# team-charls/charls

Hardware: AMD Instinct MI355X
Metric: MPixels/s encode+decode, 4096x4096 8-bit gray, bit-exact vs CharLS (higher is better)
Workload: dtype u8

## Files before the change

### charls_amd/csrc/device/tile_pipeline.hip

```cpp
#pragma once
#include <hip/hip_runtime.h>

#include <algorithm>
#include <cstdlib>

#include "pipeline_common.hip"

namespace jls {
namespace tile {

using pipe::kChains;
using pipe::kInterruptChain;
using pipe::kNoEvent;
using pipe::kStatusInvalid;
using pipe::kZeroContextChain;


constexpr uint32_t kMaxTileSamples = 8192;
constexpr uint32_t kTileLines = 16;
constexpr uint32_t kSegments = 16;
constexpr uint32_t kThreads = 512;
constexpr uint32_t kWaves = kThreads / 64;
constexpr uint32_t kPackThreads = 512;
constexpr uint16_t kNoLocalSlot = 0xFFFF;
template <typename S>
struct SlotOf
{
    typedef uint32_t type;
};
template <>
struct SlotOf<uint8_t>
{
    typedef uint16_t type;
};
template <typename S>
using Slot = typename SlotOf<S>::type;
template <typename S>
constexpr uint32_t run_slots_of()
{
    return sizeof(Slot<S>) == 2 ? 2u : 1u;
}
constexpr uint32_t kRowChainWords = 288;
constexpr uint32_t kChainPad = 32;
constexpr uint32_t kSlack = kChains * kChainPad + 128;
__host__ __device__ inline uint64_t slots_capacity(uint64_t samples, uint32_t run_slots, uint64_t lines)
{
    const uint64_t runs = samples / 2 + lines < samples ? samples / 2 + lines : samples;
    return samples + (run_slots > 1 ? runs : 0);
}
__host__ __device__ inline size_t stage_bytes(uint32_t tile_capacity, uint32_t sample_bytes)
{
    return sample_bytes == 1 ? (size_t)slots_capacity(tile_capacity, 2, kTileLines) * 2 : (size_t)tile_capacity * 4;
}
constexpr uint32_t kPlanGroups = 64;
#define JLS_HOST_DEV_EARLY __host__ __device__ inline
constexpr uint32_t kRunTag = 1u << 31;

enum Counter : uint32_t
{
    kCountJobs = 0,
    kCountJobsRewalked = 1,
    kCountRunJobs = 2,
    kCountRunJobsRewalked = 3,
    kCountRareSegments = 4,
    kCountRareSerial = 5,
// ... 175 lines not shown
        __syncthreads();
        if (lane == 63)
        {
            s_tmp[wave] = incl_a;
            s_tmp[kWaves + wave] = incl_b;
        }
        __syncthreads();
        uint32_t before_a = carry_a, before_b = carry_b, all_a = 0, all_b = 0;
        for (int w2 = 0; w2 < waves; ++w2)
        {
            const uint32_t na = s_tmp[w2], nb = s_tmp[kWaves + w2];
            before_a += w2 < wave ? na : 0;
            before_b += w2 < wave ? nb : 0;
            all_a += na;
            all_b += nb;
        }
        a[half] = before_a + incl_a - a[half];
        b[half] = before_b + incl_b - b[half];
        carry_a += all_a;
        carry_b += all_b;
    }
}

template <typename S, int ILV>
struct Samples
{
    const ScanDesc& d;
    const S* rows;
    uint32_t first_line;
    int mask;
    JLS_DEV int operator()(uint32_t line, uint32_t x) const
    {
        static_assert(ILV == 0, "planar scans only");
        return (int)rows[(size_t)(line + 1 - first_line) * d.width + x] & mask;
    }
};

template <typename S, int ILV>
JLS_DEV void stage_lines(const ScanDesc& d, const TileGeometry& g, S* rows)
{
    const uint32_t width = g.width;
    const uint32_t bytes = width * (uint32_t)sizeof(S);
    const uint32_t first = g.first_line == 0 ? 1u : 0u;
    if (first)
        for (uint32_t x = threadIdx.x; x < width; x += blockDim.x)
            rows[x] = 0;
// ... 69 lines not shown
__global__ void __launch_bounds__(kThreads) analyze_tiles(const ScanDesc* __restrict__ descs, const Work* __restrict__ works)
{
    JLS_DYNAMIC_LDS(smem);
    const ScanDesc d = descs[blockIdx.y];
    const Work w = works[blockIdx.y];
    const Traits t = make_traits(d);
    const uint32_t tile = tile_of_block(blockIdx.x, scan_tiles(d, w));
    if (tile >= scan_tiles(d, w))
        return;
    const TileGeometry g = tile_geometry(d, w, tile);
    constexpr uint32_t step = 1;
    const int lane = threadIdx.x & 63, wave = threadIdx.x >> 6;
    const uint32_t width = g.width, chunks = g.chunks;
    const TileLds lds = tile_lds<S, ILV>(width, w.lines_per_tile, true);
    S* s_rows = reinterpret_cast<S*>(smem + lds.rows);
    uint16_t* s_key = reinterpret_cast<uint16_t*>(smem + lds.keys);
    uint64_t* s_eq = reinterpret_cast<uint64_t*>(smem + lds.masks);
    uint64_t* s_q0 = s_eq + (size_t)w.lines_per_tile * chunks;
    uint32_t* s_hist = reinterpret_cast<uint32_t*>(smem + lds.table);
    unsigned char* s_grad = reinterpret_cast<unsigned char*>(s_hist + kChains + 1);
    const int mask = (1 << d.bits_per_sample) - 1;
    const Samples<S, ILV> sample{d, s_rows, g.first_line, mask};

    stage_lines<S, ILV>(d, g, s_rows);
    for (uint32_t c = threadIdx.x; c < (uint32_t)kChains; c += kThreads)
        s_hist[c] = 0;
    if (sizeof(S) == 1)
        for (uint32_t q = threadIdx.x; q < 511; q += kThreads)
            s_grad[q] = (unsigned char)(quantize(t, (int)q - 255) + 4);
    __syncthreads();

    for (uint32_t sgm = wave; sgm < g.segments; sgm += kWaves)
    {
        const uint32_t r = sgm / g.pieces, piece = sgm % g.pieces;
        const uint32_t y = g.first_line + r;
        const uint32_t k0 = piece * g.chunks_per_piece;
        const uint32_t k1 = k0 + g.chunks_per_piece < chunks ? k0 + g.chunks_per_piece : chunks;
        const int edge_a = y >= step ? sample(y - step, 0) : 0;
        const int edge_c = y >= 2 * step ? (r >= 1 ? sample(y - 2 * step, 0) : pipe::load_sample<S, 0>(d, y - 2, 0, mask)) : 0;
        for (uint32_t k = k0; k < k1; ++k)
        {
            const uint32_t x = k * 64 + lane;
            bool eq = false, q0 = false;
            if (x < width)
            {
                const int v = sample(y, x);
                const int ra = x > 0 ? sample(y, x - 1) : edge_a;
                int rb = 0, rc = 0, rd = 0;
                if (y >= step)
                {
                    rb = sample(y - step, x);
                    rc = x > 0 ? sample(y - step, x - 1) : edge_c;
                    rd = sample(y - step, x + 1 < width ? x + 1 : width - 1);
                }
                else
                    rc = x > 0 ? 0 : edge_c;
                const int qs = sizeof(S) == 1
                                   ? ((int)s_grad[rd - rb + 255] * 9 + (int)s_grad[rb - rc + 255]) * 9 + (int)s_grad[rc - ra + 255] - 364
                                   : context_id(t, ra, rb, rc, rd);
                const int sg = qs >> 31;
                const int ctx = (qs ^ sg) - sg;
                s_key[r * width + x] = (uint16_t)(ctx | ((sg & 1) << 9));
                eq = v == ra;
                q0 = qs == 0;
            }
            const unsigned long long m_eq = __ballot(eq);
            const unsigned long long m_q0 = __ballot(q0);
            if (lane == 0)
            {
                s_eq[r * chunks + k] = m_eq;
                s_q0[r * chunks + k] = m_q0;
            }
        }
    }
    __syncthreads();
    for (uint32_t sgm = wave; sgm < g.segments; sgm += kWaves)
    {
        const uint32_t r = sgm / g.pieces, piece = sgm % g.pieces;
        const uint32_t y = g.first_line + r;
        const uint32_t k0 = piece * g.chunks_per_piece;
        const uint32_t k1 = k0 + g.chunks_per_piece < chunks ? k0 + g.chunks_per_piece : chunks;
        const auto key_row = global_ptr(w.keyinv) + (size_t)y * width;
        unsigned long long carry = 0;
        for (uint32_t k = 0; k < k1; ++k)
        {
            const unsigned long long a = s_eq[r * chunks + k];
            const unsigned long long b = a & s_q0[r * chunks + k];
            const unsigned long long sum = a + b + carry;
            const unsigned long long st = sum ^ a ^ b;
            carry = (((a & b) | ((a | b) & st)) >> 63) & 1ull;
            const uint32_t x = k * 64 + lane;
            if (k >= k0 && x < width)
            {
                const bool s = (st >> lane) & 1ull;
                const bool q0 = (s_q0[r * chunks + k] >> lane) & 1ull;
                const bool eq = (a >> lane) & 1ull;
                uint16_t key = s_key[r * width + x];
                if (!(s || q0))
                    atomicAdd(&s_hist[key & 0x1FF], 1u);
                else if (s && eq)
                    key = kNoEvent;
                else if (s)
                {
                    key = (uint16_t)kInterruptChain;
                    atomicAdd(&s_hist[kInterruptChain], 1u);
                }
                else
                {
                    key = 0;
                    atomicAdd(&s_hist[0], 1u);
                }
                key_row[x] = key;
            }
        }
    }
    __syncthreads();
    for (uint32_t c = threadIdx.x; c < (uint32_t)kChains; c += kThreads)
        global_ptr(w.seg)[(size_t)tile * kChains + c] = s_hist[c];
}

constexpr uint32_t kPlanThreads = 384;
JLS_DEV void plan_group(const ScanDesc& d, const Work& w, uint32_t g, uint32_t& t0, uint32_t& t1)
{
    const uint32_t tiles = scan_tiles(d, w);
    const uint32_t per_group = (tiles + kPlanGroups - 1) / kPlanGroups;
    t0 = g * per_group < tiles ? g * per_group : tiles;
    t1 = t0 + per_group < tiles ? t0 + per_group : tiles;
}
__global__ void __launch_bounds__(kPlanThreads) sum_chains(const ScanDesc* __restrict__ descs, const Work* __restrict__ works)
{
    const ScanDesc d = descs[blockIdx.y];
    const Work w = works[blockIdx.y];
    const uint32_t g = blockIdx.x, c = threadIdx.x;
    if (c >= (uint32_t)kChains)
        return;
    uint32_t t0, t1;
    plan_group(d, w, g, t0, t1);
    uint32_t sum = 0;
    for (uint32_t t = t0; t < t1; ++t)
        sum += w.seg[(size_t)t * kChains + c];
    w.plan_part[g * kChains + c] = sum * (c == 0 ? w.run_slots : 1u);
// ... 105 lines not shown
    static JLS_DEV int err(uint32_t v) { return (int)(v << (32 - kRunBits - kErrBits)) >> (32 - kErrBits); }
    static JLS_DEV int which(uint32_t v) { return (int)((v >> (kRunBits + kErrBits)) & 1u); }
    static JLS_DEV uint32_t component(uint32_t v) { return (v >> (is_end_of_line(v) ? 15u : kRunBits + kErrBits + 1)) & 3u; }
};

template <typename S, int ILV>
__global__ void __launch_bounds__(kThreads) sort_tiles(const ScanDesc* __restrict__ descs, const Work* __restrict__ works)
{
    JLS_DYNAMIC_LDS(smem);
    const ScanDesc d = descs[blockIdx.y];
    const Work w = works[blockIdx.y];
    const Traits t = make_traits(d);
    const uint32_t tile = tile_of_block(blockIdx.x, scan_tiles(d, w));
    if (tile >= scan_tiles(d, w))
        return;
    const TileGeometry g = tile_geometry(d, w, tile);
    constexpr uint32_t step = 1;
    const int lane = threadIdx.x & 63, wave = threadIdx.x >> 6;
    const uint32_t width = g.width, chunks = g.chunks;
    const TileLds lds = tile_lds<S, ILV>(width, w.lines_per_tile, false);
    S* s_rows = reinterpret_cast<S*>(smem + lds.rows);
    uint64_t* s_noev = reinterpret_cast<uint64_t*>(smem + lds.masks);
    uint32_t* s_lead = reinterpret_cast<uint32_t*>(s_noev + (size_t)w.lines_per_tile * chunks);
    uint32_t* s_segoff = reinterpret_cast<uint32_t*>(smem + lds.table);
    uint32_t* s_tileoff = s_segoff + sort_segments(w.lines_per_tile) * kChains;
    uint32_t* s_count = s_tileoff + kChains + 1;
    uint32_t* s_global = s_count + kChains + 1;
    uint32_t* s_tmp = s_global + kChains + 1;
    uint32_t* s_same = s_tmp + 16;
    uint32_t* s_rowbase = s_same + kWaves * (kChains + 1);
    uint16_t* s_rowchain = reinterpret_cast<uint16_t*>(s_rowbase + kChains + 1);
    Slot<S>* s_stage = reinterpret_cast<Slot<S>*>(s_rowbase + kChains + 1 + kRowChainWords);
    const int mask = (1 << d.bits_per_sample) - 1;
    const Samples<S, ILV> sample{d, s_rows, g.first_line, mask};
    const auto key_tile = global_ptr(w.keyinv) + (size_t)g.first_line * width;

    JLS_PHASE_BEGIN();
    stage_lines<S, ILV>(d, g, s_rows);
    JLS_PHASE(0);
    for (uint32_t i = threadIdx.x; i < g.segments * (uint32_t)kChains; i += kThreads)
        s_segoff[i] = 0;
    for (uint32_t i = threadIdx.x; i < kWaves * ((uint32_t)kChains + 1); i += kThreads)
        s_same[i] = 0;
    __syncthreads();
    JLS_PHASE(1);
    const bool keys_kept = g.segments <= kWaves && g.chunks_per_piece <= 16;
    uint32_t keys2[8];
#pragma unroll
    for (int i = 0; i < 8; ++i)
        keys2[i] = 0xFFFFFFFFu;
    auto fetch_keys = [&](uint32_t r, uint32_t kb, uint32_t k1) {
        uint32_t held[16];
#pragma unroll
        for (int j = 0; j < 16; ++j)
        {
            const uint32_t x = (kb + j) * 64 + lane;
            held[j] = key_tile[(size_t)r * width + (x < width ? x : width - 1)];
        }
#pragma unroll
        for (int j = 0; j < 16; ++j)
            if (!(kb + j < k1 && (kb + j) * 64 + lane < width))
                held[j] = kNoEvent;
#pragma unroll
        for (int i = 0; i < 8; ++i)
            keys2[i] = held[2 * i] | (held[2 * i + 1] << 16);
    };
// ... 34 lines not shown
            const bool full = m == ~0ull;
            const uint32_t own = full ? 64u : (uint32_t)__ffsll(~m) - 1;
            const unsigned long long rest = __ballot(full) >> lane;
            const uint32_t ones = rest == ~0ull ? 64u : (uint32_t)__ffsll(~rest) - 1;
            const uint32_t next = __shfl(own, (int)((lane + ones) & 63u));
            const uint32_t lead = 64u * ones + ((uint32_t)lane + ones < 64u ? next : behind);
            if (k < chunks)
                s_lead[r * (chunks + 1) + k] = lead;
            behind = __shfl(lead, 0);
            if (k0 == 0)
                break;
        }
        if (lane == 0)
            s_lead[r * (chunks + 1) + chunks] = 0;
    }
    {
        static_assert(kChains <= kThreads, "a chain per thread");
        const uint32_t c = threadIdx.x;
        const bool chain = c < (uint32_t)kChains;
        uint32_t n = 0;
        if (chain)
            for (uint32_t sgm = 0; sgm < g.segments; ++sgm)
                n += s_segoff[sgm * kChains + c];
        const uint32_t rows = chain && c != (uint32_t)kInterruptChain ? (n + 63) / 64 : 0u;
        uint32_t off[2] = {n, 0}, row_base[2] = {rows, 0};
        block_exclusive_scan_pair(off, row_base, kChains, s_tmp);
        if (chain)
        {
            s_tileoff[c] = off[0];
            s_count[c] = n;
            s_global[c] = global_ptr(w.seg)[(size_t)tile * kChains + c];
            uint32_t running = off[0];
            for (uint32_t sgm = 0; sgm < g.segments; ++sgm)
            {
                const uint32_t m = s_segoff[sgm * kChains + c];
                s_segoff[sgm * kChains + c] = running;
                running += m;
            }
            s_rowbase[c] = row_base[0];
            for (uint32_t j = 0; j < rows; ++j)
                s_rowchain[row_base[0] + j] = (uint16_t)c;
            if (c == (uint32_t)kChains - 1)
                s_rowbase[kChains] = row_base[0] + rows;
        }
    }
    JLS_PHASE(4);
    __syncthreads();
    JLS_PHASE(5);
    for (uint32_t sgm = wave; sgm < g.segments; sgm += kWaves)
    {
        const uint32_t r = sgm / g.pieces, piece = sgm % g.pieces;
        const uint32_t y = g.first_line + r;
        const uint32_t k0 = piece * g.chunks_per_piece;
        const uint32_t k1 = k0 + g.chunks_per_piece < chunks ? k0 + g.chunks_per_piece : chunks;
        uint32_t* segoff = s_segoff + sgm * kChains;
        uint32_t* same_of = s_same + (uint32_t)wave * (kChains + 1);
        const auto inv_row = key_tile + (size_t)r * width;
        const S* cur = s_rows + (r + 1) * width;
        const int edge_a = y >= step ? sample(y - step, 0) : 0;
        const int edge_c = y >= 2 * step ? (r >= 1 ? sample(y - 2 * step, 0) : pipe::load_sample<S, 0>(d, y - 2, 0, mask)) : 0;
        const uint32_t lane_bit = 1u << (lane & 31), below = lane_bit - 1u;
        const bool upper = lane >= 32;
        const uint32_t run_first = segoff[0];
        for (uint32_t kb = k0; kb < k1; kb += 16)
        {
            if (!keys_kept)
// ... 84 lines not shown
                    record = RunRecord<S>::end_of_line(run, 0u);
                else
                {
                    const int xv = sample(y, xi);
                    const int ia = xi > 0 ? sample(y, xi - 1) : edge_a;
                    const int ib = y >= step ? sample(y - step, xi) : 0;
                    const int which = ia == ib ? 1 : 0;
                    const int err = which ? error_value(t, xv - ia) : error_value(t, (xv - ib) * ((ib - ia) < 0 ? -1 : 1));
                    record = RunRecord<S>::interrupted(run, err, which, 0u);
                }
                if (run_slots_of<S>() == 2)
                {
                    s_stage[slot] = (Slot<S>)(record & 0xFFFFu);
                    s_stage[slot + 1] = (Slot<S>)(record >> 16);
                }
                else
                    s_stage[slot] = (Slot<S>)record;
            }
        }
    }
    JLS_PHASE(6);
    __syncthreads();
    JLS_PHASE(7);
    const uint32_t total_rows = s_rowbase[kChains];
    constexpr int kRows = 4;
    for (uint32_t q0 = (uint32_t)wave * kRows; q0 < total_rows; q0 += kWaves * kRows)
    {
        uint32_t to[kRows];
        Slot<S> held[kRows];
        bool live[kRows];
#pragma unroll
        for (int j = 0; j < kRows; ++j)
        {
            const uint32_t q = q0 + (uint32_t)j;
            const uint32_t c = q < total_rows ? s_rowchain[q] : 0u;
            const uint32_t i = (q - s_rowbase[c]) * 64 + (uint32_t)lane;
            live[j] = q < total_rows && i < s_count[c];
            to[j] = s_global[c] + i;
            held[j] = live[j] ? s_stage[s_tileoff[c] + i] : (Slot<S>)0;
        }
#pragma unroll
        for (int j = 0; j < kRows; ++j)
            if (live[j])
                global_ptr(rec_slots<S>(w))[to[j]] = held[j];
    }
    JLS_PHASE(8);
}

}
}
#include "tile_pixel_mode.hip"
namespace jls {
namespace tile {

struct Chain
{
    int a, b, c, n;
    uint32_t bad;
};

JLS_DEV int chain_n_before(uint32_t i, uint32_t reset)
{
    if (reset == 0 || i < reset)
        return (int)(i + 1);
    const uint32_t half = reset >> 1, period = reset - half;
    return (int)(half + 1 + (i - reset) % period);
}

// ... 779 lines not shown
    for (uint32_t j = 1; j < jobs; ++j)
    {
        const RunJob cur = w.run_jobs[j];
        RunState out = cur.out;
        if (!same_state(cur.in, prev))
        {
            ++rewalked;
            out = prev;
            const uint32_t from = j * w.run_job_events;
            const uint32_t to = from + w.run_job_events < n ? from + w.run_job_events : n;
            walk_runs<S, ILV, true, FMT>(t, runs, run_code, int_code, from, to, out, cur.type0, cur.type1, cur.own_slot, int_rec, nc);
        }
        prev = out;
    }
    atomicAdd(&w.counters[kCountRunJobs], jobs);
    if (rewalked)
        atomicAdd(&w.counters[kCountRunJobsRewalked], rewalked);
}

#define JLS_HOST_DEV __host__ __device__ inline
JLS_HOST_DEV uint32_t pack_bits_offset(uint32_t tile_capacity, uint32_t sample_bytes)
{
    const uint32_t codes = (uint32_t)stage_bytes(tile_capacity, sample_bytes);
    const uint32_t head = ((codes + 3u) & ~3u) + 4 * ((uint32_t)kChains + 1) * 4 + kPackThreads * 4 + 16 * 4 + kRowChainWords * 4;
    return (head + 15u) & ~15u;
}

JLS_HOST_DEV uint32_t pack_bits_words(uint32_t tile_capacity, int32_t bits_per_sample)
{
    const uint32_t limit = 2u * (uint32_t)(bits_per_sample + (bits_per_sample > 8 ? bits_per_sample : 8));
    return tile_capacity * limit / 32 + 2;
}

JLS_DEV void expand_code(uint32_t word, uint64_t& bits, int& len)
{
    if (word & kRunTag)
    {
        const int ones = (int)((word >> 25) & 63u), tail_len = (int)((word >> 20) & 31u);
        bits = ((((uint64_t)1 << ones) - 1ull) << tail_len) | (uint64_t)(word & 0xFFFFFu);
        len = ones + tail_len;
    }
    else
    {
        bits = word & 0xFFFFFFu;
        len = (int)(word >> 24);
    }
}

// ... 3 lines not shown
        return bits[i];
    return (i == 0 ? carry : bits[i - 1] << (32u - head)) | (bits[i] >> head);
}

typedef uint32_t UnalignedWords4 __attribute__((vector_size(16), aligned(2)));
template <typename S>
__global__ void __launch_bounds__(kPackThreads) pack_tiles(const ScanDesc* __restrict__ descs, const Work* __restrict__ works)
{
    JLS_DYNAMIC_LDS(smem);
    constexpr bool kNarrow = sizeof(Slot<S>) == 2;
    const ScanDesc d = descs[blockIdx.y];
    const Work w = works[blockIdx.y];
    const uint32_t tile = blockIdx.x;
    const uint32_t tiles = scan_tiles(d, w);
    if (tile >= tiles)
        return;
    const uint32_t tile_capacity = w.tile_capacity;
    const uint32_t threads = blockDim.x;
    const uint32_t per_thread = ((tile_capacity + threads - 1) / threads + 7u) & ~7u;
    const int lane = threadIdx.x & 63, wave = threadIdx.x >> 6;
    const uint32_t kPackWaves = threads / 64;
    Slot<S>* s_code = reinterpret_cast<Slot<S>*>(smem);
    const uint32_t code_bytes = (uint32_t)stage_bytes(tile_capacity, (uint32_t)sizeof(S));
    uint32_t* s_tileoff = reinterpret_cast<uint32_t*>(smem + ((code_bytes + 3u) & ~3u));
    uint32_t* s_count = s_tileoff + kChains + 1;
    uint32_t* s_global = s_count + kChains + 1;
    uint32_t* s_scan = s_global + kChains + 1;
    uint32_t* s_tmp = s_scan + kPackThreads;
    uint32_t* s_rowbase = s_tmp + 16;
    uint16_t* s_rowchain = reinterpret_cast<uint16_t*>(s_rowbase + kChains + 1);
    uint32_t* s_bits = reinterpret_cast<uint32_t*>(smem + pack_bits_offset(tile_capacity, (uint32_t)sizeof(S)));
    const TileSpan span = tile_span(d, w, tile);
    const uint32_t tile_samples = span.count;
    const auto inv = global_ptr(w.keyinv) + span.first;

    constexpr int kGroups = (int)(kMaxTileSamples / kPackThreads / 8);
    uint4 mine[kGroups];
    JLS_PHASE_BEGIN();
#pragma unroll
    for (int q = 0; q < kGroups; ++q)
    {
        const uint32_t at = threadIdx.x * per_thread + (uint32_t)q * 8;
        mine[q] = make_uint4(~0u, ~0u, ~0u, ~0u);
        if ((uint32_t)q * 8 < per_thread && at + 8 <= tile_samples)
        {
            const UnalignedWords4 v = *reinterpret_cast<const JLS_GLOBAL_AS UnalignedWords4*>(inv + at);
            mine[q] = make_uint4(v[0], v[1], v[2], v[3]);
        }
        else if ((uint32_t)q * 8 < per_thread && at < tile_samples)
        {
            uint32_t e[8];
#pragma unroll
            for (int j = 0; j < 8; ++j)
                e[j] = at + (uint32_t)j < tile_samples ? inv[at + j] : kNoLocalSlot;
            mine[q] = make_uint4(e[0] | (e[1] << 16), e[2] | (e[3] << 16), e[4] | (e[5] << 16), e[6] | (e[7] << 16));
        }
    }
    {
        uint32_t n[2] = {0, 0}, g[2] = {0, 0}, rows[2] = {0, 0};
        for (int half = 0; half < 2; ++half)
        {
            const uint32_t c = threadIdx.x + (uint32_t)half * threads;
            if (c < (uint32_t)kChains)
            {
                g[half] = global_ptr(w.seg)[(size_t)tile * kChains + c];
                n[half] = global_ptr(w.seg)[(size_t)(tile + 1) * kChains + c] - g[half];
                rows[half] = (n[half] + 63) / 64;
            }
        }
        uint32_t off[2] = {n[0], n[1]}, row_base[2] = {rows[0], rows[1]};
        block_exclusive_scan_pair(off, row_base, kChains, s_tmp);
        for (int half = 0; half < 2; ++half)
        {
            const uint32_t c = threadIdx.x + (uint32_t)half * threads;
            if (c < (uint32_t)kChains)
            {
                s_tileoff[c] = off[half];
                s_count[c] = n[half];
                s_global[c] = g[half];
                s_rowbase[c] = row_base[half];
                for (uint32_t j = 0; j < rows[half]; ++j)
                    s_rowchain[row_base[half] + j] = (uint16_t)c;
                if (c == (uint32_t)kChains - 1)
                    s_rowbase[kChains] = row_base[half] + rows[half];
            }
        }
    }
    JLS_PHASE(9);
    __syncthreads();
    JLS_PHASE(11);
    {
        const uint32_t total_rows = s_rowbase[kChains];
        constexpr int kRows = 16;
        for (uint32_t q0 = (uint32_t)wave * kRows; q0 < total_rows; q0 += kPackWaves * kRows)
        {
            uint32_t to[kRows];
            Slot<S> held[kRows];
            bool live[kRows];
#pragma unroll
            for (int j = 0; j < kRows; ++j)
            {
                const uint32_t q = q0 + (uint32_t)j;
                const uint32_t c = q < total_rows ? s_rowchain[q] : 0u;
                const uint32_t i = (q - s_rowbase[c]) * 64 + (uint32_t)lane;
                live[j] = q < total_rows && i < s_count[c];
                to[j] = s_tileoff[c] + i;
                held[j] = live[j] ? global_ptr(code_slots<S>(w))[s_global[c] + i] : (Slot<S>)0;
            }
#pragma unroll
            for (int j = 0; j < kRows; ++j)
                if (live[j])
                    s_code[to[j]] = held[j];
        }
    }
    JLS_PHASE(12);
    __syncthreads();
    JLS_PHASE(13);

    auto slot_of = [&](int q, int j) -> uint32_t {
        const uint32_t word = (j >> 1) == 0 ? mine[q].x : (j >> 1) == 1 ? mine[q].y : (j >> 1) == 2 ? mine[q].z : mine[q].w;
        return (j & 1) ? word >> 16 : word & 0xFFFFu;
    };
    const uint32_t run_slots_end = kNarrow ? s_count[0] : 0u;
    auto word_of = [&](uint32_t slot) -> uint32_t {
        if (slot == kNoLocalSlot)
            return 0u;
        if (!kNarrow)
            return (uint32_t)s_code[slot];
        if (slot < run_slots_end)
            return (uint32_t)s_code[slot] | ((uint32_t)s_code[slot + 1] << 16);
        const uint32_t c = (uint32_t)s_code[slot];
        return ((c >> 10) << 24) | (c & 0x3FFu);
    };
    uint32_t words[kGroups * 8];
    uint32_t sum = 0;
#pragma unroll
    for (int q = 0; q < kGroups; ++q)
#pragma unroll
        for (int j = 0; j < 8; ++j)
        {
            const uint32_t word = word_of(slot_of(q, j));
            words[q * 8 + j] = word;
            sum += word & kRunTag ? ((word >> 25) & 63u) + ((word >> 20) & 31u) : word >> 24;
        }
    JLS_PHASE(14);
    {
// ... 148 lines not shown
}

__global__ void __launch_bounds__(256) clear_pack_state(const Work* __restrict__ works, uint32_t bytes_per_scan)
{
    uint4* at = reinterpret_cast<uint4*>(works[blockIdx.y].blockbase);
    const uint32_t groups = bytes_per_scan / 16;
    for (uint32_t g = blockIdx.x * 256u + threadIdx.x; g < groups; g += gridDim.x * 256u)
        at[g] = make_uint4(0, 0, 0, 0);
}

inline size_t tile_common_lds_bytes(uint32_t width, uint32_t lines_per_tile, uint32_t sample_bytes, int interleave_mode, bool with_keys)
{
    auto up = [](size_t v) { return (v + 15) & ~size_t{15}; };
    const size_t chunks = (width + 63) / 64;
    return up(interleave_mode == 1 ? 0 : (size_t)(lines_per_tile + 1) * width * sample_bytes) +
           (with_keys ? up((size_t)lines_per_tile * width * 2) : 0) + up((size_t)lines_per_tile * chunks * 16);
}
inline size_t analyze_lds_bytes(uint32_t width, uint32_t lines_per_tile, uint32_t sample_bytes, int interleave_mode)
{
    return tile_common_lds_bytes(width, lines_per_tile, sample_bytes, interleave_mode, true) + ((size_t)kChains + 1) * 4 + pipe::kGradientTable;
}
inline size_t sort_lds_bytes(uint32_t width, uint32_t lines_per_tile, uint32_t sample_bytes, int interleave_mode)
{
    return tile_common_lds_bytes(width, lines_per_tile, sample_bytes, interleave_mode, false) + (size_t)sort_segments(lines_per_tile) * kChains * 4 +
           4 * ((size_t)kChains + 1) * 4 + 16 * 4 + (size_t)kWaves * (kChains + 1) * 4 + kRowChainWords * 4 +
           stage_bytes((uint32_t)lines_per_tile * width, sample_bytes);
}
inline uint32_t pack_threads_for(uint32_t tile_capacity)
{
    const uint32_t per_thread = ((tile_capacity + kPackThreads - 1) / kPackThreads + 7u) & ~7u;
    if ((uint64_t)per_thread * kPackThreads * 4 <= (uint64_t)tile_capacity * 5)
        return kPackThreads;
    const uint32_t fewer = ((tile_capacity + per_thread - 1) / per_thread + 63u) / 64u * 64u;
    return fewer < 192u ? 192u : (fewer > kPackThreads ? kPackThreads : fewer);
}
inline size_t pack_lds_bytes(uint32_t tile_capacity, int32_t bits_per_sample)
{
    return (size_t)pack_bits_offset(tile_capacity, bits_per_sample > 8 ? 2u : 1u) + (size_t)pack_bits_words(tile_capacity, bits_per_sample) * 4;
}
struct TilePlan
{
    uint32_t mode, nc, step, lines, line_samples, lines_per_tile, segs_per_line, seg_pixels, tiles, tile_capacity, max_pixels;
    uint64_t samples;
};
inline TilePlan plan_tiles(const ScanDesc& d)
{
    TilePlan p{};
    const uint32_t sample_bytes = d.bits_per_sample > 8 ? 2u : 1u;
// ... 35 lines not shown
```

### charls_amd/csrc/device/tile_pixel_mode.hip

```cpp
#pragma once

namespace jls {
namespace tile {

struct RunRecord2
{
    static constexpr uint32_t kEol = 1u << 31, kZero = 1u << 30;
    static JLS_DEV uint32_t end_of_line(uint32_t run, uint32_t component) { return run | (component << 28) | kEol; }
    static JLS_DEV uint32_t interrupted(uint32_t run, int which, uint32_t component) { return run | ((uint32_t)which << 27) | (component << 28); }
    static JLS_DEV uint32_t zero_run(int err, int which, uint32_t component)
    {
        return ((uint32_t)err & 0x1FFFFu) | ((uint32_t)which << 27) | (component << 28) | kZero;
    }
    static JLS_DEV uint32_t interruption(int err) { return (uint32_t)err & 0x1FFFFu; }
    static JLS_DEV bool is_end_of_line(uint32_t v) { return (v >> 31) != 0; }
    static JLS_DEV bool is_zero_run(uint32_t v) { return ((v >> 30) & 1u) != 0; }
    static JLS_DEV uint32_t run(uint32_t v) { return is_zero_run(v) ? 0u : v & 0x7FFFFFFu; }
    static JLS_DEV uint32_t component(uint32_t v) { return (v >> 28) & 3u; }
    static JLS_DEV int err(uint32_t v) { return (int)(v << 15) >> 15; }
    static JLS_DEV int which(uint32_t v) { return (int)((v >> 27) & 1u); }
};
template <typename S>
JLS_DEV int interruption_err(Slot<S> v)
{
// ... 444 lines not shown

template <typename S>
__global__ void __launch_bounds__(kThreads) sort_pixel_tiles(const ScanDesc* __restrict__ descs, const Work* __restrict__ works)
{
    JLS_DYNAMIC_LDS(smem);
    const ScanDesc d = descs[blockIdx.y];
    const Work w = works[blockIdx.y];
    const Traits t = make_traits(d);
    const uint32_t tile = tile_of_block(blockIdx.x, scan_tiles(d, w));
    if (tile >= scan_tiles(d, w))
        return;
    const PixelTile g = pixel_tile(d, w, tile);
    const int lane = threadIdx.x & 63, wave = threadIdx.x >> 6;
    const uint32_t nc = g.nc;
    const uint32_t Ps = g.pixels * nc;
    const uint32_t max_pixels = tile_row_pixels(d.width, w.segs_per_line, w.seg_pixels);
    const uint32_t max_chunks = (max_pixels * nc + 63) / 64, chunks = (Ps + 63) / 64;
    const uint32_t chunks_per_piece = (chunks + g.pieces - 1) / g.pieces;
    const uint32_t segments = g.tile_lines * g.pieces;
    const PixelLds lds = pixel_lds(w.lines_per_tile, g.step, max_pixels, nc, (uint32_t)sizeof(S), w.tile_capacity, false, max_chunks);
    S* s_rows = reinterpret_cast<S*>(smem + lds.rows);
    uint64_t* s_noev = reinterpret_cast<uint64_t*>(smem + lds.masks);
    uint32_t* s_lead = reinterpret_cast<uint32_t*>(s_noev + (size_t)w.lines_per_tile * max_chunks);
    uint32_t* s_segoff = reinterpret_cast<uint32_t*>(smem + lds.table);
    uint32_t* s_tileoff = s_segoff + sort_segments(w.lines_per_tile) * kChains;
    uint32_t* s_count = s_tileoff + kChains + 1;
    uint32_t* s_global = s_count + kChains + 1;
    uint32_t* s_tmp = s_global + kChains + 1;
    uint32_t* s_same = s_tmp + 16;
    uint32_t* s_rowbase = s_same + kWaves * (kChains + 1);
    uint16_t* s_rowchain = reinterpret_cast<uint16_t*>(s_rowbase + kChains + 1);
    Slot<S>* s_stage = reinterpret_cast<Slot<S>*>(s_rowbase + kChains + 1 + kRowChainWords);
    const int mask = (1 << d.bits_per_sample) - 1;
    auto key_row = [&](uint32_t r) -> uint16_t* { return w.keyinv + (size_t)(g.first_line + r) * g.line_samples + (size_t)g.px0 * nc; };

    stage_pixel_rows<S>(d, g, s_rows, mask);
    for (uint32_t i = threadIdx.x; i < segments * (uint32_t)kChains; i += kThreads)
        s_segoff[i] = 0;
    for (uint32_t i = threadIdx.x; i < kWaves * ((uint32_t)kChains + 1); i += kThreads)
        s_same[i] = 0;
    __syncthreads();
    for (uint32_t sgm = wave; sgm < segments; sgm += kWaves)
    {
        const uint32_t r = sgm / g.pieces, piece = sgm % g.pieces;
        const uint32_t k0 = piece * chunks_per_piece;
        const uint32_t k1 = k0 + chunks_per_piece < chunks ? k0 + chunks_per_piece : chunks;
        const uint16_t* keys = key_row(r);
        for (uint32_t kb = k0; kb < k1; kb += 16)
        {
            uint16_t held[16];
#pragma unroll
            for (int j = 0; j < 16; ++j)
            {
                const uint32_t q = (kb + j) * 64 + lane;
                held[j] = kb + j < k1 && q < Ps ? keys[q] : kNoEvent;
            }
#pragma unroll
            for (int j = 0; j < 16; ++j)
            {
                const uint32_t k = kb + j;
                if (k < k1)
                {
                    const uint32_t q = k * 64 + lane;
                    const uint16_t key = held[j];
                    if (q < Ps && key != kNoEvent)
                        atomicAdd(&s_segoff[sgm * kChains + (key & 0x1FF)], (key & 0x1FF) == 0 ? run_slots_of<S>() : 1u);
                    const unsigned long long m = __ballot(q < Ps && key == kNoEvent);
                    if (lane == 0)
                        s_noev[r * max_chunks + k] = m;
                }
            }
        }
    }
    __syncthreads();
    {
        uint32_t n[2] = {0, 0};
        for (int half = 0; half < 2; ++half)
        {
            const uint32_t c = threadIdx.x + (uint32_t)half * kThreads;
            if (c < (uint32_t)kChains)
                for (uint32_t sgm = 0; sgm < segments; ++sgm)
                    n[half] += s_segoff[sgm * kChains + c];
        }
        uint32_t off[2] = {n[0], n[1]};
        block_exclusive_scan(off[0], off[1], s_tmp);
        for (int half = 0; half < 2; ++half)
        {
            const uint32_t c = threadIdx.x + (uint32_t)half * kThreads;
            if (c < (uint32_t)kChains)
            {
                s_tileoff[c] = off[half];
                s_count[c] = n[half];
                s_global[c] = w.seg[(size_t)tile * kChains + c];
                uint32_t running = off[half];
                for (uint32_t sgm = 0; sgm < segments; ++sgm)
                {
                    const uint32_t m = s_segoff[sgm * kChains + c];
                    s_segoff[sgm * kChains + c] = running;
                    running += m;
                }
            }
        }
        uint32_t rows[2], row_base[2];
        for (int half = 0; half < 2; ++half)
        {
            const uint32_t c = threadIdx.x + (uint32_t)half * kThreads;
            rows[half] = row_base[half] = c < (uint32_t)kChains ? (n[half] + 63) / 64 : 0u;
        }
        block_exclusive_scan(row_base[0], row_base[1], s_tmp);
        for (int half = 0; half < 2; ++half)
        {
            const uint32_t c = threadIdx.x + (uint32_t)half * kThreads;
            if (c < (uint32_t)kChains)
            {
                s_rowbase[c] = row_base[half];
                for (uint32_t j = 0; j < rows[half]; ++j)
                    s_rowchain[row_base[half] + j] = (uint16_t)c;
                if (c == (uint32_t)kChains - 1)
                    s_rowbase[kChains] = row_base[half] + rows[half];
            }
        }
        if (threadIdx.x >= kThreads - g.tile_lines)
        {
            const uint32_t r = kThreads - 1 - threadIdx.x;
            uint32_t lead = 0;
            s_lead[r * (max_chunks + 1) + chunks] = 0;
            for (uint32_t k = chunks; k-- > 0;)
            {
                const unsigned long long m = s_noev[r * max_chunks + k];
                lead = m == ~0ull ? 64 + lead : (uint32_t)__ffsll(~m) - 1;
                s_lead[r * (max_chunks + 1) + k] = lead;
            }
        }
    }
    __syncthreads();
    for (uint32_t sgm = wave; sgm < segments; sgm += kWaves)
    {
        const uint32_t r = sgm / g.pieces, piece = sgm % g.pieces;
        const uint32_t y = g.first_line + r;
        const uint32_t k0 = piece * chunks_per_piece;
        const uint32_t k1 = k0 + chunks_per_piece < chunks ? k0 + chunks_per_piece : chunks;
        uint32_t* segoff = s_segoff + sgm * kChains;
// ... 84 lines not shown
                    {
                        int above[4] = {0, 0, 0, 0};
                        if (nc == 1 && y >= g.step)
                            load_coded_pixel<S>(d, y - g.step, x + run, mask, above);
                        record = RunRecord2::interrupted(run, nc == 1 && v == above[0] ? 1 : 0, component);
                    }
                }
            }
            if (has)
            {
                if (run_slots_of<S>() == 2 && chain == 0)
                {
                    s_stage[slot] = (Slot<S>)(record & 0xFFFFu);
                    s_stage[slot + 1] = (Slot<S>)(record >> 16);
                }
                else
                    s_stage[slot] = (Slot<S>)record;
            }
            if (inside)
                inv_row[q] = has ? (uint16_t)slot : kNoLocalSlot;
        }
    }
    __syncthreads();
    const uint32_t total_rows = s_rowbase[kChains];
    for (uint32_t q0 = (uint32_t)wave * 4; q0 < total_rows; q0 += kWaves * 4)
    {
        uint32_t to[4];
        Slot<S> held[4];
        bool live[4];
#pragma unroll
        for (int j = 0; j < 4; ++j)
        {
            const uint32_t q = q0 + (uint32_t)j;
            const uint32_t c = q < total_rows ? s_rowchain[q] : 0u;
            const uint32_t i = (q - s_rowbase[c]) * 64 + (uint32_t)lane;
            live[j] = q < total_rows && i < s_count[c];
            to[j] = s_global[c] + i;
            held[j] = live[j] ? s_stage[s_tileoff[c] + i] : (Slot<S>)0;
        }
#pragma unroll
        for (int j = 0; j < 4; ++j)
            if (live[j])
                rec_slots<S>(w)[to[j]] = held[j];
    }
}

inline size_t analyze_pixel_lds_bytes(uint32_t lines_per_tile, uint32_t step, uint32_t max_pixels, uint32_t nc, uint32_t sample_bytes, uint32_t tile_capacity)
{
    const PixelLds l = pixel_lds(lines_per_tile, step, max_pixels, nc, sample_bytes, tile_capacity, true, (max_pixels + 63) / 64);
    return (size_t)l.table + ((size_t)kChains + 1) * 4 + pipe::kGradientTable + 16;
}
inline size_t sort_pixel_lds_bytes(uint32_t lines_per_tile, uint32_t step, uint32_t max_pixels, uint32_t nc, uint32_t sample_bytes, uint32_t tile_capacity)
{
    const PixelLds l = pixel_lds(lines_per_tile, step, max_pixels, nc, sample_bytes, tile_capacity, false, (max_pixels * nc + 63) / 64);
    return (size_t)l.table + (size_t)sort_segments(lines_per_tile) * kChains * 4 + 4 * ((size_t)kChains + 1) * 4 + 16 * 4 +
           (size_t)kWaves * (kChains + 1) * 4 + kRowChainWords * 4 + stage_bytes(tile_capacity, sample_bytes);
}

}
}
```

Baseline: 16960.

## Replace per-chain row tables with dense piece tables for scatter and gather copies

The copy loops between the LDS stage and global slot buffers in the sort, pixel-mode sort and pack kernels now walk the tile's packed samples densely in 64-wide rows. Each lane finds its chain piece through a per-row base index plus a start-bit mask counted with mbcnt. Before, rows were padded per chain and needed rowchain and rowbase lookups, so many lanes sat idle on partial rows. The change also drops the tileoff, count and global arrays and adds a piece table sized for the maximum tile, which raises LDS use. Phase markers are added to the analyze kernel.

```diff
diff --git a/charls_amd/csrc/device/tile_pipeline.hip b/charls_amd/csrc/device/tile_pipeline.hip
--- a/charls_amd/csrc/device/tile_pipeline.hip
+++ b/charls_amd/csrc/device/tile_pipeline.hip
@@ -40,7 +40,6 @@
 {
     return sizeof(Slot<S>) == 2 ? 2u : 1u;
 }
-constexpr uint32_t kRowChainWords = 288;
 constexpr uint32_t kChainPad = 32;
 constexpr uint32_t kSlack = kChains * kChainPad + 128;
 __host__ __device__ inline uint64_t slots_capacity(uint64_t samples, uint32_t run_slots, uint64_t lines)
@@ -262,6 +261,98 @@
     }
 }
 
+constexpr uint32_t kPieceRows = (kMaxTileSamples + kMaxTileSamples / 2 + kTileLines + 63) / 64;
+constexpr uint32_t kPieceInfo = 4;
+constexpr uint32_t kPieceWords = kChains + kPieceInfo;
+constexpr uint32_t kNoPiece = 0xFFFFFFFFu;
+enum PieceInfo : uint32_t
+{
+    kPieceTotal = 0,
+    kPieceSkip = 1,
+    kPieceRun = 2
+};
+JLS_DEV void piece_tables_clear(uint4* rows, uint32_t* pieces)
+{
+    for (uint32_t r = threadIdx.x; r < kPieceRows; r += blockDim.x)
+        rows[r] = make_uint4(0, 0, 0, 0);
+    if (threadIdx.x < kPieceInfo)
+        pieces[kChains + threadIdx.x] = threadIdx.x == kPieceSkip ? kNoPiece : 0u;
+}
+JLS_DEV void piece_tables_add(uint4* rows, uint32_t* pieces, uint32_t k, uint32_t off, uint32_t n, uint32_t global)
+{
+    uint32_t* words = reinterpret_cast<uint32_t*>(rows);
+    pieces[k] = global - off;
+    const uint32_t j = off & 63u;
+    if (j != 0)
+        atomicOr(&words[(off >> 6) * 4 + 2 + ((j - 1) >> 5)], 1u << ((j - 1) & 31u));
+    for (uint32_t r = (off + 63) >> 6; r * 64 < off + n; ++r)
+        words[r * 4] = k;
+}
+JLS_DEV uint32_t piece_of_lane(const uint4& e, int lane)
+{
+#ifdef JLS_EMULATED
+    const unsigned long long starts = (unsigned long long)e.z | ((unsigned long long)e.w << 32);
+    return e.x + (uint32_t)__popcll(starts & ((1ull << lane) - 1ull));
+#else
+    (void)lane;
+    return e.x + __builtin_amdgcn_mbcnt_hi(e.w, __builtin_amdgcn_mbcnt_lo(e.z, 0u));
+#endif
+}
+template <typename T, int kRows>
+JLS_DEV void copy_pieces_out(const uint4* rows, const uint32_t* pieces, const T* from, JLS_GLOBAL_AS T* to, uint32_t waves)
+{
+    const int lane = threadIdx.x & 63, wave = threadIdx.x >> 6;
+    const uint32_t total = pieces[kChains + kPieceTotal], skip = pieces[kChains + kPieceSkip];
+    const uint32_t total_rows = (total + 63) / 64;
+    for (uint32_t q0 = (uint32_t)wave * kRows; q0 < total_rows; q0 += waves * kRows)
+    {
+        uint32_t at[kRows];
+        T held[kRows];
+        bool live[kRows];
+#pragma unroll
+        for (int j = 0; j < kRows; ++j)
+        {
+            const uint32_t q = q0 + (uint32_t)j < total_rows ? q0 + (uint32_t)j : total_rows - 1;
+            const uint32_t t = q * 64 + (uint32_t)lane;
+            const uint32_t k = piece_of_lane(rows[q], lane);
+            const uint32_t tc = t < total ? t : total - 1;
+            live[j] = q0 + (uint32_t)j < total_rows && t < total && k != skip;
+            at[j] = tc + pieces[k];
+            held[j] = from[tc];
+        }
+#pragma unroll
+        for (int j = 0; j < kRows; ++j)
+            if (live[j])
+                to[at[j]] = held[j];
+    }
+}
+template <typename T, int kRows>
+JLS_DEV void copy_pieces_in(const uint4* rows, const uint32_t* pieces, const JLS_GLOBAL_AS T* from, T* to, uint32_t waves)
+{
+    const int lane = threadIdx.x & 63, wave = threadIdx.x >> 6;
+    const uint32_t total = pieces[kChains + kPieceTotal];
+    const uint32_t total_rows = (total + 63) / 64;
+    for (uint32_t q0 = (uint32_t)wave * kRows; q0 < total_rows; q0 += waves * kRows)
+    {
+        T held[kRows];
+#pragma unroll
+        for (int j = 0; j < kRows; ++j)
+        {
+            const uint32_t q = q0 + (uint32_t)j < total_rows ? q0 + (uint32_t)j : total_rows - 1;
+            const uint32_t t = q * 64 + (uint32_t)lane;
+            const uint32_t k = piece_of_lane(rows[q], lane);
+            held[j] = from[(t < total ? t : total - 1) + pieces[k]];
+        }
+#pragma unroll
+        for (int j = 0; j < kRows; ++j)
+        {
+            const uint32_t t = (q0 + (uint32_t)j) * 64 + (uint32_t)lane;
+            if (t < total)
+                to[t] = held[j];
+        }
+    }
+}
+
 template <typename S, int ILV>
 struct Samples
 {
@@ -377,13 +468,16 @@
     const int mask = (1 << d.bits_per_sample) - 1;
     const Samples<S, ILV> sample{d, s_rows, g.first_line, mask};
 
+    JLS_PHASE_BEGIN();
     stage_lines<S, ILV>(d, g, s_rows);
+    JLS_PHASE(22);
     for (uint32_t c = threadIdx.x; c < (uint32_t)kChains; c += kThreads)
         s_hist[c] = 0;
     if (sizeof(S) == 1)
         for (uint32_t q = threadIdx.x; q < 511; q += kThreads)
             s_grad[q] = (unsigned char)(quantize(t, (int)q - 255) + 4);
     __syncthreads();
+    JLS_PHASE(23);
 
     for (uint32_t sgm = wave; sgm < g.segments; sgm += kWaves)
     {
@@ -428,7 +522,9 @@
             }
         }
     }
+    JLS_PHASE(24);
     __syncthreads();
+    JLS_PHASE(25);
     for (uint32_t sgm = wave; sgm < g.segments; sgm += kWaves)
     {
         const uint32_t r = sgm / g.pieces, piece = sgm % g.pieces;
@@ -469,9 +565,11 @@
             }
         }
     }
+    JLS_PHASE(26);
     __syncthreads();
     for (uint32_t c = threadIdx.x; c < (uint32_t)kChains; c += kThreads)
         global_ptr(w.seg)[(size_t)tile * kChains + c] = s_hist[c];
+    JLS_PHASE(27);
 }
 
 constexpr uint32_t kPlanThreads = 384;
@@ -623,15 +721,12 @@
     S* s_rows = reinterpret_cast<S*>(smem + lds.rows);
     uint64_t* s_noev = reinterpret_cast<uint64_t*>(smem + lds.masks);
     uint32_t* s_lead = reinterpret_cast<uint32_t*>(s_noev + (size_t)w.lines_per_tile * chunks);
-    uint32_t* s_segoff = reinterpret_cast<uint32_t*>(smem + lds.table);
-    uint32_t* s_tileoff = s_segoff + sort_segments(w.lines_per_tile) * kChains;
-    uint32_t* s_count = s_tileoff + kChains + 1;
-    uint32_t* s_global = s_count + kChains + 1;
-    uint32_t* s_tmp = s_global + kChains + 1;
+    uint4* s_piecerows = reinterpret_cast<uint4*>(smem + lds.table);
+    uint32_t* s_segoff = reinterpret_cast<uint32_t*>(s_piecerows + kPieceRows);
+    uint32_t* s_tmp = s_segoff + sort_segments(w.lines_per_tile) * kChains;
     uint32_t* s_same = s_tmp + 16;
-    uint32_t* s_rowbase = s_same + kWaves * (kChains + 1);
-    uint16_t* s_rowchain = reinterpret_cast<uint16_t*>(s_rowbase + kChains + 1);
-    Slot<S>* s_stage = reinterpret_cast<Slot<S>*>(s_rowbase + kChains + 1 + kRowChainWords);
+    uint32_t* s_pieces = s_same + kWaves * (kChains + 1);
+    Slot<S>* s_stage = reinterpret_cast<Slot<S>*>(s_pieces + kPieceWords);
     const int mask = (1 << d.bits_per_sample) - 1;
     const Samples<S, ILV> sample{d, s_rows, g.first_line, mask};
     const auto key_tile = global_ptr(w.keyinv) + (size_t)g.first_line * width;
@@ -643,6 +738,7 @@
         s_segoff[i] = 0;
     for (uint32_t i = threadIdx.x; i < kWaves * ((uint32_t)kChains + 1); i += kThreads)
         s_same[i] = 0;
+    piece_tables_clear(s_piecerows, s_pieces);
     __syncthreads();
     JLS_PHASE(1);
     const bool keys_kept = g.segments <= kWaves && g.chunks_per_piece <= 16;
@@ -723,14 +819,19 @@
         if (chain)
             for (uint32_t sgm = 0; sgm < g.segments; ++sgm)
                 n += s_segoff[sgm * kChains + c];
-        const uint32_t rows = chain && c != (uint32_t)kInterruptChain ? (n + 63) / 64 : 0u;
-        uint32_t off[2] = {n, 0}, row_base[2] = {rows, 0};
-        block_exclusive_scan_pair(off, row_base, kChains, s_tmp);
+        const uint32_t global = chain ? global_ptr(w.seg)[(size_t)tile * kChains + c] : 0u;
+        uint32_t off[2] = {n, 0}, piece[2] = {n != 0 ? 1u : 0u, 0};
+        block_exclusive_scan_pair(off, piece, kChains, s_tmp);
         if (chain)
         {
-            s_tileoff[c] = off[0];
-            s_count[c] = n;
-            s_global[c] = global_ptr(w.seg)[(size_t)tile * kChains + c];
+            if (n != 0)
+            {
+                piece_tables_add(s_piecerows, s_pieces, piece[0], off[0], n, global);
+                if (c == (uint32_t)kInterruptChain)
+                    s_pieces[kChains + kPieceSkip] = piece[0];
+            }
+            if (c == (uint32_t)kChains - 1)
+                s_pieces[kChains + kPieceTotal] = off[0] + n;
             uint32_t running = off[0];
             for (uint32_t sgm = 0; sgm < g.segments; ++sgm)
             {
@@ -738,11 +839,6 @@
                 s_segoff[sgm * kChains + c] = running;
                 running += m;
             }
-            s_rowbase[c] = row_base[0];
-            for (uint32_t j = 0; j < rows; ++j)
-                s_rowchain[row_base[0] + j] = (uint16_t)c;
-            if (c == (uint32_t)kChains - 1)
-                s_rowbase[kChains] = row_base[0] + rows;
         }
     }
     JLS_PHASE(4);
@@ -873,28 +969,7 @@
     JLS_PHASE(6);
     __syncthreads();
     JLS_PHASE(7);
-    const uint32_t total_rows = s_rowbase[kChains];
-    constexpr int kRows = 4;
-    for (uint32_t q0 = (uint32_t)wave * kRows; q0 < total_rows; q0 += kWaves * kRows)
-    {
-        uint32_t to[kRows];
-        Slot<S> held[kRows];
-        bool live[kRows];
-#pragma unroll
-        for (int j = 0; j < kRows; ++j)
-        {
-            const uint32_t q = q0 + (uint32_t)j;
-            const uint32_t c = q < total_rows ? s_rowchain[q] : 0u;
-            const uint32_t i = (q - s_rowbase[c]) * 64 + (uint32_t)lane;
-            live[j] = q < total_rows && i < s_count[c];
-            to[j] = s_global[c] + i;
-            held[j] = live[j] ? s_stage[s_tileoff[c] + i] : (Slot<S>)0;
-        }
-#pragma unroll
-        for (int j = 0; j < kRows; ++j)
-            if (live[j])
-                global_ptr(rec_slots<S>(w))[to[j]] = held[j];
-    }
+    copy_pieces_out<Slot<S>, 4>(s_piecerows, s_pieces, s_stage, global_ptr(rec_slots<S>(w)), kWaves);
     JLS_PHASE(8);
 }
 
@@ -1720,8 +1795,8 @@
 JLS_HOST_DEV uint32_t pack_bits_offset(uint32_t tile_capacity, uint32_t sample_bytes)
 {
     const uint32_t codes = (uint32_t)stage_bytes(tile_capacity, sample_bytes);
-    const uint32_t head = ((codes + 3u) & ~3u) + 4 * ((uint32_t)kChains + 1) * 4 + kPackThreads * 4 + 16 * 4 + kRowChainWords * 4;
-    return (head + 15u) & ~15u;
+    const uint32_t head = ((codes + 3u) & ~3u) + kPackThreads * 4 + 16 * 4 + kPieceWords * 4;
+    return ((head + 15u) & ~15u) + kPieceRows * 16;
 }
 
 JLS_HOST_DEV uint32_t pack_bits_words(uint32_t tile_capacity, int32_t bits_per_sample)
@@ -1771,14 +1846,12 @@
     const uint32_t kPackWaves = threads / 64;
     Slot<S>* s_code = reinterpret_cast<Slot<S>*>(smem);
     const uint32_t code_bytes = (uint32_t)stage_bytes(tile_capacity, (uint32_t)sizeof(S));
-    uint32_t* s_tileoff = reinterpret_cast<uint32_t*>(smem + ((code_bytes + 3u) & ~3u));
-    uint32_t* s_count = s_tileoff + kChains + 1;
-    uint32_t* s_global = s_count + kChains + 1;
-    uint32_t* s_scan = s_global + kChains + 1;
+    uint32_t* s_scan = reinterpret_cast<uint32_t*>(smem + ((code_bytes + 3u) & ~3u));
     uint32_t* s_tmp = s_scan + kPackThreads;
-    uint32_t* s_rowbase = s_tmp + 16;
-    uint16_t* s_rowchain = reinterpret_cast<uint16_t*>(s_rowbase + kChains + 1);
-    uint32_t* s_bits = reinterpret_cast<uint32_t*>(smem + pack_bits_offset(tile_capacity, (uint32_t)sizeof(S)));
+    uint32_t* s_pieces = s_tmp + 16;
+    const uint32_t bits_offset = pack_bits_offset(tile_capacity, (uint32_t)sizeof(S));
+    uint4* s_piecerows = reinterpret_cast<uint4*>(smem + bits_offset) - kPieceRows;
+    uint32_t* s_bits = reinterpret_cast<uint32_t*>(smem + bits_offset);
     const TileSpan span = tile_span(d, w, tile);
     const uint32_t tile_samples = span.count;
     const auto inv = global_ptr(w.keyinv) + span.first;
@@ -1805,8 +1878,9 @@
             mine[q] = make_uint4(e[0] | (e[1] << 16), e[2] | (e[3] << 16), e[4] | (e[5] << 16), e[6] | (e[7] << 16));
         }
     }
-    {
-        uint32_t n[2] = {0, 0}, g[2] = {0, 0}, rows[2] = {0, 0};
+    piece_tables_clear(s_piecerows, s_pieces);
+    {
+        uint32_t n[2] = {0, 0}, g[2] = {0, 0};
         for (int half = 0; half < 2; ++half)
         {
             const uint32_t c = threadIdx.x + (uint32_t)half * threads;
@@ -1814,54 +1888,28 @@
             {
                 g[half] = global_ptr(w.seg)[(size_t)tile * kChains + c];
                 n[half] = global_ptr(w.seg)[(size_t)(tile + 1) * kChains + c] - g[half];
-                rows[half] = (n[half] + 63) / 64;
-            }
-        }
-        uint32_t off[2] = {n[0], n[1]}, row_base[2] = {rows[0], rows[1]};
-        block_exclusive_scan_pair(off, row_base, kChains, s_tmp);
+            }
+        }
+        uint32_t off[2] = {n[0], n[1]}, piece[2] = {n[0] != 0 ? 1u : 0u, n[1] != 0 ? 1u : 0u};
+        block_exclusive_scan_pair(off, piece, kChains, s_tmp);
         for (int half = 0; half < 2; ++half)
         {
             const uint32_t c = threadIdx.x + (uint32_t)half * threads;
             if (c < (uint32_t)kChains)
             {
-                s_tileoff[c] = off[half];
-                s_count[c] = n[half];
-                s_global[c] = g[half];
-                s_rowbase[c] = row_base[half];
-                for (uint32_t j = 0; j < rows[half]; ++j)
-                    s_rowchain[row_base[half] + j] = (uint16_t)c;
+                if (n[half] != 0)
+                    piece_tables_add(s_piecerows, s_pieces, piece[half], off[half], n[half], g[half]);
+                if (c == 0)
+                    s_pieces[kChains + kPieceRun] = n[half];
                 if (c == (uint32_t)kChains - 1)
-                    s_rowbase[kChains] = row_base[half] + rows[half];
+                    s_pieces[kChains + kPieceTotal] = off[half] + n[half];
             }
         }
     }
     JLS_PHASE(9);
     __syncthreads();
     JLS_PHASE(11);
-    {
-        const uint32_t total_rows = s_rowbase[kChains];
-        constexpr int kRows = 16;
-        for (uint32_t q0 = (uint32_t)wave * kRows; q0 < total_rows; q0 += kPackWaves * kRows)
-        {
-            uint32_t to[kRows];
-            Slot<S> held[kRows];
-            bool live[kRows];
-#pragma unroll
-            for (int j = 0; j < kRows; ++j)
-            {
-                const uint32_t q = q0 + (uint32_t)j;
-                const uint32_t c = q < total_rows ? s_rowchain[q] : 0u;
-                const uint32_t i = (q - s_rowbase[c]) * 64 + (uint32_t)lane;
-                live[j] = q < total_rows && i < s_count[c];
-                to[j] = s_tileoff[c] + i;
-                held[j] = live[j] ? global_ptr(code_slots<S>(w))[s_global[c] + i] : (Slot<S>)0;
-            }
-#pragma unroll
-            for (int j = 0; j < kRows; ++j)
-                if (live[j])
-                    s_code[to[j]] = held[j];
-        }
-    }
+    copy_pieces_in<Slot<S>, 16>(s_piecerows, s_pieces, global_ptr(code_slots<S>(w)), s_code, kPackWaves);
     JLS_PHASE(12);
     __syncthreads();
     JLS_PHASE(13);
@@ -1870,7 +1918,7 @@
         const uint32_t word = (j >> 1) == 0 ? mine[q].x : (j >> 1) == 1 ? mine[q].y : (j >> 1) == 2 ? mine[q].z : mine[q].w;
         return (j & 1) ? word >> 16 : word & 0xFFFFu;
     };
-    const uint32_t run_slots_end = kNarrow ? s_count[0] : 0u;
+    const uint32_t run_slots_end = kNarrow ? s_pieces[kChains + kPieceRun] : 0u;
     auto word_of = [&](uint32_t slot) -> uint32_t {
         if (slot == kNoLocalSlot)
             return 0u;
@@ -2065,8 +2113,8 @@
 }
 inline size_t sort_lds_bytes(uint32_t width, uint32_t lines_per_tile, uint32_t sample_bytes, int interleave_mode)
 {
-    return tile_common_lds_bytes(width, lines_per_tile, sample_bytes, interleave_mode, false) + (size_t)sort_segments(lines_per_tile) * kChains * 4 +
-           4 * ((size_t)kChains + 1) * 4 + 16 * 4 + (size_t)kWaves * (kChains + 1) * 4 + kRowChainWords * 4 +
+    return tile_common_lds_bytes(width, lines_per_tile, sample_bytes, interleave_mode, false) + (size_t)kPieceRows * 16 +
+           (size_t)sort_segments(lines_per_tile) * kChains * 4 + 16 * 4 + (size_t)kWaves * (kChains + 1) * 4 + (size_t)kPieceWords * 4 +
            stage_bytes((uint32_t)lines_per_tile * width, sample_bytes);
 }
 inline uint32_t pack_threads_for(uint32_t tile_capacity)
diff --git a/charls_amd/csrc/device/tile_pixel_mode.hip b/charls_amd/csrc/device/tile_pixel_mode.hip
--- a/charls_amd/csrc/device/tile_pixel_mode.hip
+++ b/charls_amd/csrc/device/tile_pixel_mode.hip
@@ -490,15 +490,12 @@
     S* s_rows = reinterpret_cast<S*>(smem + lds.rows);
     uint64_t* s_noev = reinterpret_cast<uint64_t*>(smem + lds.masks);
     uint32_t* s_lead = reinterpret_cast<uint32_t*>(s_noev + (size_t)w.lines_per_tile * max_chunks);
-    uint32_t* s_segoff = reinterpret_cast<uint32_t*>(smem + lds.table);
-    uint32_t* s_tileoff = s_segoff + sort_segments(w.lines_per_tile) * kChains;
-    uint32_t* s_count = s_tileoff + kChains + 1;
-    uint32_t* s_global = s_count + kChains + 1;
-    uint32_t* s_tmp = s_global + kChains + 1;
+    uint4* s_piecerows = reinterpret_cast<uint4*>(smem + lds.table);
+    uint32_t* s_segoff = reinterpret_cast<uint32_t*>(s_piecerows + kPieceRows);
+    uint32_t* s_tmp = s_segoff + sort_segments(w.lines_per_tile) * kChains;
     uint32_t* s_same = s_tmp + 16;
-    uint32_t* s_rowbase = s_same + kWaves * (kChains + 1);
-    uint16_t* s_rowchain = reinterpret_cast<uint16_t*>(s_rowbase + kChains + 1);
-    Slot<S>* s_stage = reinterpret_cast<Slot<S>*>(s_rowbase + kChains + 1 + kRowChainWords);
+    uint32_t* s_pieces = s_same + kWaves * (kChains + 1);
+    Slot<S>* s_stage = reinterpret_cast<Slot<S>*>(s_pieces + kPieceWords);
     const int mask = (1 << d.bits_per_sample) - 1;
     auto key_row = [&](uint32_t r) -> uint16_t* { return w.keyinv + (size_t)(g.first_line + r) * g.line_samples + (size_t)g.px0 * nc; };
 
@@ -507,6 +504,7 @@
         s_segoff[i] = 0;
     for (uint32_t i = threadIdx.x; i < kWaves * ((uint32_t)kChains + 1); i += kThreads)
         s_same[i] = 0;
+    piece_tables_clear(s_piecerows, s_pieces);
     __syncthreads();
     for (uint32_t sgm = wave; sgm < segments; sgm += kWaves)
     {
@@ -550,16 +548,17 @@
                 for (uint32_t sgm = 0; sgm < segments; ++sgm)
                     n[half] += s_segoff[sgm * kChains + c];
         }
-        uint32_t off[2] = {n[0], n[1]};
-        block_exclusive_scan(off[0], off[1], s_tmp);
+        uint32_t off[2] = {n[0], n[1]}, piece[2] = {n[0] != 0 ? 1u : 0u, n[1] != 0 ? 1u : 0u};
+        block_exclusive_scan_pair(off, piece, kChains, s_tmp);
         for (int half = 0; half < 2; ++half)
         {
             const uint32_t c = threadIdx.x + (uint32_t)half * kThreads;
             if (c < (uint32_t)kChains)
             {
-                s_tileoff[c] = off[half];
-                s_count[c] = n[half];
-                s_global[c] = w.seg[(size_t)tile * kChains + c];
+                if (n[half] != 0)
+                    piece_tables_add(s_piecerows, s_pieces, piece[half], off[half], n[half], w.seg[(size_t)tile * kChains + c]);
+                if (c == (uint32_t)kChains - 1)
+                    s_pieces[kChains + kPieceTotal] = off[half] + n[half];
                 uint32_t running = off[half];
                 for (uint32_t sgm = 0; sgm < segments; ++sgm)
                 {
@@ -567,25 +566,6 @@
                     s_segoff[sgm * kChains + c] = running;
                     running += m;
                 }
-            }
-        }
-        uint32_t rows[2], row_base[2];
-        for (int half = 0; half < 2; ++half)
-        {
-            const uint32_t c = threadIdx.x + (uint32_t)half * kThreads;
-            rows[half] = row_base[half] = c < (uint32_t)kChains ? (n[half] + 63) / 64 : 0u;
-        }
-        block_exclusive_scan(row_base[0], row_base[1], s_tmp);
-        for (int half = 0; half < 2; ++half)
-        {
-            const uint32_t c = threadIdx.x + (uint32_t)half * kThreads;
-            if (c < (uint32_t)kChains)
-            {
-                s_rowbase[c] = row_base[half];
-                for (uint32_t j = 0; j < rows[half]; ++j)
-                    s_rowchain[row_base[half] + j] = (uint16_t)c;
-                if (c == (uint32_t)kChains - 1)
-                    s_rowbase[kChains] = row_base[half] + rows[half];
             }
         }
         if (threadIdx.x >= kThreads - g.tile_lines)
@@ -716,27 +696,7 @@
         }
     }
     __syncthreads();
-    const uint32_t total_rows = s_rowbase[kChains];
-    for (uint32_t q0 = (uint32_t)wave * 4; q0 < total_rows; q0 += kWaves * 4)
-    {
-        uint32_t to[4];
-        Slot<S> held[4];
-        bool live[4];
-#pragma unroll
-        for (int j = 0; j < 4; ++j)
-        {
-            const uint32_t q = q0 + (uint32_t)j;
-            const uint32_t c = q < total_rows ? s_rowchain[q] : 0u;
-            const uint32_t i = (q - s_rowbase[c]) * 64 + (uint32_t)lane;
-            live[j] = q < total_rows && i < s_count[c];
-            to[j] = s_global[c] + i;
-            held[j] = live[j] ? s_stage[s_tileoff[c] + i] : (Slot<S>)0;
-        }
-#pragma unroll
-        for (int j = 0; j < 4; ++j)
-            if (live[j])
-                rec_slots<S>(w)[to[j]] = held[j];
-    }
+    copy_pieces_out<Slot<S>, 4>(s_piecerows, s_pieces, s_stage, global_ptr(rec_slots<S>(w)), kWaves);
 }
 
 inline size_t analyze_pixel_lds_bytes(uint32_t lines_per_tile, uint32_t step, uint32_t max_pixels, uint32_t nc, uint32_t sample_bytes, uint32_t tile_capacity)
@@ -747,9 +707,9 @@
 inline size_t sort_pixel_lds_bytes(uint32_t lines_per_tile, uint32_t step, uint32_t max_pixels, uint32_t nc, uint32_t sample_bytes, uint32_t tile_capacity)
 {
     const PixelLds l = pixel_lds(lines_per_tile, step, max_pixels, nc, sample_bytes, tile_capacity, false, (max_pixels * nc + 63) / 64);
-    return (size_t)l.table + (size_t)sort_segments(lines_per_tile) * kChains * 4 + 4 * ((size_t)kChains + 1) * 4 + 16 * 4 +
-           (size_t)kWaves * (kChains + 1) * 4 + kRowChainWords * 4 + stage_bytes(tile_capacity, sample_bytes);
-}
-
-}
-}
+    return (size_t)l.table + (size_t)kPieceRows * 16 + (size_t)sort_segments(lines_per_tile) * kChains * 4 + 16 * 4 +
+           (size_t)kWaves * (kChains + 1) * 4 + (size_t)kPieceWords * 4 + stage_bytes(tile_capacity, sample_bytes);
+}
+
+}
+}
```

Result: faster. 17340 (median of 6 runs) (+2.2%).
